# drdeford/FlipComplexityEmpirical

Hardware: AMD Instinct MI355X
Metric: flip steps/sec (whole node), 100×100 grid k=4 batched chains; % HBM peak (higher is better)
Workload: dtype int32

## Files before the change

### flipcomplexityempirical_amd/csrc/fw_grid16.hip

```cpp
#include <hip/hip_runtime.h>

#include <cstdio>
#include <cstdlib>

#include <algorithm>

#include "fw_device.h"

#ifdef FW_STAMPS
__device__ unsigned long long g_stamps[16];
__device__ unsigned long long g_unit_t[2 * 65536];
__device__ unsigned long long g_unit_hw[65536];
#define UNIT_TIME(u, e)                                                         \
  do {                                                                          \
    uint64_t t_;                                                                \
    asm volatile("s_memrealtime %0\n\ts_waitcnt lgkmcnt(0)" : "=s"(t_)::"memory"); \
    if (__lane_id() == 0 && (u) < 65536) {                                      \
      g_unit_t[2 * (u) + (e)] = t_;                                             \
      if ((e) == 0)                                                             \
        g_unit_hw[u] = (unsigned long long)__builtin_amdgcn_s_getreg((31 << 11) | 4) | \
                       ((unsigned long long)__builtin_amdgcn_s_getreg((31 << 11) | 20) << 32); \
    }                                                                           \
  } while (0)
#define STAMP_DECL uint64_t st_acc[16] = {}; uint64_t st_t0 = 0;
#define STAMP(i)                                              \
  do {                                                        \
    __builtin_amdgcn_sched_barrier(0);                        \
    uint64_t st_t1;                                           \
    asm volatile("s_memtime %0\n\ts_waitcnt lgkmcnt(0)" : "=s"(st_t1)::"memory"); \
    __builtin_amdgcn_sched_barrier(0);                        \
    if (i >= 0) st_acc[(i) < 0 ? 0 : (i)] += st_t1 - st_t0;   \
    st_t0 = st_t1;                                            \
  } while (0)
#define STAMP_FLUSH                                           \
  if (__lane_id() == 0)                                       \
    for (int i_ = 0; i_ < 16; ++i_) atomicAdd(&g_stamps[i_], (unsigned long long)st_acc[i_]);
#define STAMP_COUNT(i, v) st_acc[i] += (uint64_t)(v)
#else
#define STAMP_COUNT(i, v)
#define STAMP_DECL
#define STAMP(i)
#define STAMP_FLUSH
#define UNIT_TIME(u, e)
#endif

#include <cstddef>

static_assert(sizeof(fw_chain_stats) == 136, "fw_chain_stats layout");
static_assert(offsetof(fw_chain_stats, yields) == 88 && offsetof(fw_chain_stats, sum_invb) == 112 &&
                  offsetof(fw_chain_stats, cut) == 120 && offsetof(fw_chain_stats, npairs) == 128,
              "fw_chain_stats layout");

#define HIST_ADD(ptr, v) atomicAdd(ptr, v)

void* fw_grid16_pick_lean(int lb, int mode, int G, bool w4);
void* fw_grid16_pick_w2(int mode, int G, bool w4);

namespace {

constexpr int ROW = 16;
constexpr int MAX_NW = 4;
constexpr uint32_t SCR_BLOCK = 15;
constexpr int LDS_GUARD = 16;

struct Hood16 {
  int x;
  uint32_t lx;
  uint32_t bits;
  uint32_t cnt;
  bool has_v;
  int deg;
};

struct GDiv {
  uint32_t m, s;
  __device__ __forceinline__ int operator()(int x) const {
    return (int)(__umul24((uint32_t)x, m) >> s);
  }
};
__device__ __forceinline__ int mulW(int r, int W) { return (int)__umul24((uint32_t)r, (uint32_t)W); }

__device__ __forceinline__ uint32_t rowbits(uint64_t bal, int row) {
  return (uint32_t)(bal >> (row * ROW)) & 0xFFFFu;
}
__device__ __forceinline__ uint32_t row_scan(uint32_t x) {
  x += (uint32_t)__builtin_amdgcn_update_dpp(0, (int)x, 0x111, 0xF, 0xF, true);
  x += (uint32_t)__builtin_amdgcn_update_dpp(0, (int)x, 0x112, 0xF, 0xF, true);
  x += (uint32_t)__builtin_amdgcn_update_dpp(0, (int)x, 0x114, 0xF, 0xF, true);
  x += (uint32_t)__builtin_amdgcn_update_dpp(0, (int)x, 0x118, 0xF, 0xF, true);
  return x;
}
__device__ __forceinline__ uint32_t row_last(uint32_t x) {
  return (uint32_t)__builtin_amdgcn_update_dpp(0, (int)x, 0x15F, 0xF, 0xF, false);
}
__device__ __forceinline__ uint32_t row_sum(uint32_t x) { return row_last(row_scan(x)); }
__device__ __forceinline__ uint32_t row_first(uint32_t x) {
  return (uint32_t)__builtin_amdgcn_update_dpp(0, (int)x, 0x150, 0xF, 0xF, false);
}
__device__ __forceinline__ uint32_t row_shl1(uint32_t x) {
  return (uint32_t)__builtin_amdgcn_update_dpp(0, (int)x, 0x101, 0xF, 0xF, false);
}
__device__ __forceinline__ uint32_t row_pick(uint32_t x, int L, int q) {
  const int src = ((__lane_id() - q) + L) << 2;
  return (uint32_t)__builtin_amdgcn_ds_bpermute(src, (int)x);
}

template <int LB>
__device__ __forceinline__ uint32_t lab_window(const LDS uint8_t* lab, int x) {
  const int bit = (x - 1) * LB;
  const int wi = bit >> 5;
  const LDS uint32_t* w = reinterpret_cast<const LDS uint32_t*>(lab);
  const uint32_t lo0 = w[wi];
  const uint32_t lo = wi >= 0 ? lo0 : 0u;
  const uint32_t hi = w[wi + 1];
  const uint64_t both = ((uint64_t)hi << 32) | lo;
  return (uint32_t)(both >> (uint32_t)(bit - wi * 32)) & ((1u << (6 * LB)) - 1u);
}

template <int LB, int MODE>
__device__ __forceinline__ void weights4(const LDS uint8_t* lab, int x0, int W, int H, int n,
                                         GDiv gd, uint32_t& w4, uint32_t& cd4) {
  constexpr uint32_t M = (1u << LB) - 1u;
  w4 = 0;
  cd4 = 0;
  if (x0 >= n) return;
  const uint32_t own = lab_window<LB>(lab, x0);
  const uint32_t up = x0 + 3 - W >= 0 ? lab_window<LB>(lab, x0 - W) : 0u;
  const uint32_t dn = x0 + W < n ? lab_window<LB>(lab, x0 + W) : 0u;
  const int r0 = gd(x0);
  const int c0 = x0 - mulW(r0, W);
#pragma unroll
  for (int tt = 0; tt < 4; ++tt) {
    int ct = c0 + tt, rt = r0;
    if (ct >= W) {
      ct -= W;
      rt += 1;
    }
    const uint32_t lx = (own >> (LB * (tt + 1))) & M;
    const uint32_t ll = (own >> (LB * tt)) & M;
    const uint32_t lr = (own >> (LB * (tt + 2))) & M;
    const uint32_t lu = (up >> (LB * (tt + 1))) & M, ld = (dn >> (LB * (tt + 1))) & M;
    uint32_t bits = 0, cd = 0;
    if (rt > 0) { bits |= 1u << lu; cd += lu != lx; }
    if (ct > 0) { bits |= 1u << ll; cd += ll != lx; }
    if (ct < W - 1) { bits |= 1u << lr; cd += lr != lx; }
    if (rt < H - 1) { bits |= 1u << ld; cd += ld != lx; }
    uint32_t w = MODE == FW_PROPOSE_CUTEDGE ? cd : (uint32_t)__popc(bits & ~(1u << lx));
    if (x0 + tt >= n) w = cd = 0;
    w4 |= w << (8 * tt);
    cd4 |= cd << (8 * tt);
  }
}

__device__ __forceinline__ uint32_t bsum4(uint32_t v) {
  return (v & 0xFFu) + ((v >> 8) & 0xFFu) + ((v >> 16) & 0xFFu) + (v >> 24);
}

__device__ __forceinline__ uint32_t spread4(uint32_t u) {
  const uint32_t t = ((u << 12) | u) & 0x000F000Fu;
  return ((t << 6) | t) & 0x03030303u;
}
__device__ __forceinline__ uint32_t onehot4(uint32_t s) {
  return __builtin_amdgcn_perm(0u, 0x08040201u, s);
}
__device__ __forceinline__ uint32_t low_bytes(int t) {
  const uint32_t tc = (uint32_t)min(max(t, 0), 4);
  return tc == 4u ? 0xFFFFFFFFu : (1u << (8u * tc)) - 1u;
}
__device__ __forceinline__ uint32_t ne_bytes(uint32_t a, uint32_t b) {
  return ~((a & b) + 0x7F7F7F7Fu) & 0x80808080u;
}
__device__ __forceinline__ uint32_t byte_popc(uint32_t f) {
  const uint32_t t = f - ((f >> 1) & 0x55555555u);
  return (t & 0x33333333u) + ((t >> 2) & 0x33333333u);
}

template <int MODE, bool NEED_CD, bool BATCH = true, bool W4 = false>
__device__ __forceinline__ void weights4_swar(const LDS uint8_t* lab, int x0, int W, int H, int n,
                                              GDiv gd, uint32_t& w4, uint32_t& cd4) {
  w4 = 0;
  cd4 = 0;
  const int xs = x0 < n ? x0 : 0;
  const bool hasU = xs + 3 - W >= 0, hasD = xs + W < n;
  const LDS uint32_t* lw32 = reinterpret_cast<const LDS uint32_t*>(lab);
  const int xw[3] = {xs, hasU ? xs - W : xs, hasD ? xs + W : xs};
  uint32_t wlo[3], whi[3];
  int wbit[3];
#pragma unroll
  for (int t = 0; t < 3; ++t) {
    wbit[t] = (xw[t] - 1) * 2;
    const int wi = wbit[t] >> 5;
    wlo[t] = lw32[wi];
    whi[t] = lw32[wi + 1];
  }
  const int r0 = gd(x0);
  const int c0 = x0 - mulW(r0, W);
  const int tw = W - c0;
  uint32_t mN, mU, mD, mL, mR;
  if constexpr (W4) {
    mN = x0 < n ? 0xFFFFFFFFu : 0u;
    mU = r0 > 0 ? 0xFFFFFFFFu : 0u;
    mD = r0 < H - 1 ? 0xFFFFFFFFu : 0u;
    mL = c0 == 0 ? 0xFFFFFF00u : 0xFFFFFFFFu;
    mR = tw == 4 ? 0x00FFFFFFu : 0xFFFFFFFFu;
  } else {
    const uint32_t t8 = (uint32_t)min(tw, 4) << 3;
    const uint32_t nxt = (uint32_t)(~0ull << t8);
    mN = low_bytes(n - x0);
    mU = r0 > 0 ? 0xFFFFFFFFu : nxt;
    mD = r0 < H - 2 ? 0xFFFFFFFFu : (r0 == H - 2 ? ~nxt : 0u);
    mL = ~((uint32_t)(0xFFull << t8) | (c0 == 0 ? 0xFFu : 0u));
    mR = ~(uint32_t)(0xFFull << (((uint32_t)min(tw, 5) << 3) - 8u));
  }
  if constexpr (BATCH) __builtin_amdgcn_sched_barrier(0);
  uint32_t win[3];
#pragma unroll
  for (int t = 0; t < 3; ++t) {
    const int wi = wbit[t] >> 5;
    const uint64_t both = ((uint64_t)whi[t] << 32) | (wi >= 0 ? wlo[t] : 0u);
    win[t] = (uint32_t)(both >> (uint32_t)(wbit[t] - wi * 32)) & 0xFFFu;
  }
  const uint32_t own = win[0];
  const uint32_t up = hasU ? win[1] : 0u, dn = hasD ? win[2] : 0u;
  const uint32_t o_lo = onehot4(spread4(own)), o_hi = onehot4(spread4(own >> 8));
  const uint32_t L = o_lo;
  const uint32_t O = __builtin_amdgcn_alignbyte(o_hi, o_lo, 1);
  const uint32_t R = __builtin_amdgcn_alignbyte(o_hi, o_lo, 2);
  const uint32_t U = onehot4(spread4(up >> 2)), Dn = onehot4(spread4(dn >> 2));
  if constexpr (MODE != FW_PROPOSE_CUTEDGE) {
    const uint32_t bits = (U & mU) | (L & mL) | (R & mR) | (Dn & mD);
    w4 = byte_popc(bits & ~O & mN);
  }
  if constexpr (NEED_CD || MODE == FW_PROPOSE_CUTEDGE) {
    const uint32_t ne = (ne_bytes(U, O) & mU) >> 7, nl = (ne_bytes(L, O) & mL) >> 7,
                   nr = (ne_bytes(R, O) & mR) >> 7, nd = (ne_bytes(Dn, O) & mD) >> 7;
    cd4 = (ne + nl + nr + nd) & mN;
    if constexpr (MODE == FW_PROPOSE_CUTEDGE) w4 = cd4;
  }
}

template <int LB, int MODE, bool NEED_CD, bool BATCH = true, bool W4 = false>
__device__ __forceinline__ void weights4x(const LDS uint8_t* lab, int x0, int W, int H, int n,
                                          GDiv gd, uint32_t& w4, uint32_t& cd4) {
  if constexpr (LB == 2)
    weights4_swar<MODE, NEED_CD, BATCH, W4>(lab, x0, W, H, n, gd, w4, cd4);
  else
    weights4<LB, MODE>(lab, x0, W, H, n, gd, w4, cd4);
}

__device__ __forceinline__ uint32_t bsum4m(uint32_t v) { return (v * 0x01010101u) >> 24; }


__device__ __forceinline__ int window_verdict8(uint64_t A, int q, int row, bool need, uint32_t& nflood) {
#ifdef FW_STAMPS
#define FLOOD_COUNT ++nflood
#else
#define FLOOD_COUNT
#endif
  constexpr uint64_t BORDER = 0x7Full | (0x7Full << 48) | 0x0001010101010101ull | 0x0040404040404040ull;
  const uint64_t src = A & ((1ull << 19) | (1ull << 26) | (1ull << 28) | (1ull << 35));
  const int sb = q == 0 ? 19 : q == 1 ? 26 : q == 2 ? 28 : 35;
  uint64_t x = (need && q < 4) ? src & (1ull << sb) : 0ull;
  if (x) {
    for (;;) {
      const uint64_t y = (x | (x << 1) | (x >> 1) | (x << 8) | (x >> 8)) & A;
      x = (y | (y << 1) | (y >> 1) | (y << 8) | (y >> 8)) & A;
      FLOOD_COUNT;
      if (x == y) break;
    }
  }
  const uint32_t full = rowbits(ballot(x != 0ull && (x & src) == src), row);
  const uint32_t closed = rowbits(ballot(x != 0ull && (x & BORDER) == 0ull), row);
  return full ? 1 : (closed ? 0 : -1);
}

__device__ __forceinline__ uint32_t from_prev_row_lane(uint32_t x) {
  return (uint32_t)__builtin_amdgcn_update_dpp(0, (int)x, 0x111, 0xF, 0xF, true);
}
__device__ __forceinline__ uint32_t from_next_row_lane(uint32_t x) {
  return (uint32_t)__builtin_amdgcn_update_dpp(0, (int)x, 0x101, 0xF, 0xF, true);
}
__device__ __forceinline__ uint32_t dilate_row(uint32_t x) {
  return x | (x << 1) | (x >> 1) | from_prev_row_lane(x) | from_next_row_lane(x);
}

template <int LB>
__device__ int grid_race_bb_row(const LDS uint8_t* lab, int n, int W, int H, int q, int row,
                                bool need, int vr, int vc, uint32_t a, uint32_t am4, uint32_t lk,
                                uint32_t& nodes, uint32_t& degs) {
  const int r = vr - 8 + q, c0 = vc - 16;
  const bool rin = (r >= 0) & (r < H);
  uint32_t A = eq_bits32<LB>(lab, n, (rin ? r : vr) * W + c0, a);
  const int lo_cut = c0 < 0 ? -c0 : 0;
  const int hi_n = W - c0;
  uint32_t cm = ~0u << lo_cut;
  if (hi_n < 32) cm &= (1u << hi_n) - 1u;
  A &= rin ? cm : 0u;
  if (q == 8) A &= ~(1u << 16);
  uint32_t E = ((q == 0) & (r > 0)) | ((q == 15) & (r < H - 1)) ? ~0u : 0u;
  if (c0 > 0) E |= 1u;
  if (c0 + 31 < W - 1) E |= 1u << 31;
  E &= A;
  uint32_t F[4];
#pragma unroll
  for (int d = 0; d < 4; ++d) {
    const int sl = d == 0 ? 7 : (d == 3 ? 9 : 8), sb = d == 1 ? 15 : (d == 2 ? 17 : 16);
    F[d] = (q == sl && ((am4 >> d) & 1u)) ? (1u << sb) : 0u;
  }
  uint32_t M = 0x8421u;
  auto unite = [&](int i, int j) {
    const uint32_t m = ((M >> (4 * i)) | (M >> (4 * j))) & 15u;
#pragma unroll
    for (int d = 0; d < 4; ++d)
      M = ((m >> d) & 1u) ? (M & ~(15u << (4 * d))) | (m << (4 * d)) : M;
  };
  if (lk & 1u) unite(0, 2);
  if (lk & 2u) unite(2, 3);
  if (lk & 4u) unite(3, 1);
  if (lk & 8u) unite(1, 0);
  auto n_classes = [&]() {
    int nc = 0;
#pragma unroll
    for (int d = 0; d < 4; ++d)
      nc += (int)(((am4 >> d) & 1u) && (__ffs((M >> (4 * d)) & 15u) - 1) == d);
    return nc;
  };
  uint32_t V = F[0] | F[1] | F[2] | F[3];
  int verdict = need ? -2 : -1;
  uint32_t P = 0;
  while (ballot(verdict == -2)) {
    const bool run = verdict == -2;
    const uint32_t lvl = F[0] | F[1] | F[2] | F[3];
    if (run && n_classes() == 1) {
      verdict = 1;
      P = V & ~lvl;
    }
    const bool esc = rowbits(ballot((lvl & E) != 0u), row) != 0u;
    if (verdict == -2 && esc) verdict = -3;
    const bool go = verdict == -2;
    uint32_t D[4], nw = 0;
#pragma unroll
    for (int d = 0; d < 4; ++d) {
      D[d] = ((am4 >> d) & 1u) ? dilate_row(F[d]) & A : 0u;
      nw |= D[d];
    }
    nw &= ~V;
#pragma unroll
    for (int i = 0; i < 4; ++i)
#pragma unroll
      for (int j = i + 1; j < 4; ++j) {
        const bool cand = go && ((am4 >> i) & 1u) && ((am4 >> j) & 1u) && !((M >> (4 * i + j)) & 1u);
        if (rowbits(ballot(cand && (D[i] & (F[j] | (D[j] & nw))) != 0u), row)) unite(i, j);
      }
    uint32_t reach = 0;
#pragma unroll
    for (int d = 0; d < 4; ++d) {
      const uint32_t fd = D[d] & nw;
      F[d] = go ? fd : F[d];
      reach |= rowbits(ballot(fd != 0u), row) ? (1u << d) : 0u;
    }
    if (go) {
      P = V;
      if (n_classes() == 1) {
        verdict = 1;
      } else {
        bool closed = false;
#pragma unroll
        for (int d = 0; d < 4; ++d)
          closed |= ((am4 >> d) & 1u) && (reach & (M >> (4 * d)) & 15u) == 0u;
        if (closed)
          verdict = 0;
        else
          V |= nw;
      }
    }
  }
  if (verdict < 0) return -1;
  const uint32_t pc = (uint32_t)__popc(P);
  uint32_t dg = pc * (uint32_t)((r > 0) + (r < H - 1) + 2);
  if (c0 <= 0) dg -= (P >> (-c0)) & 1u;
  if (hi_n <= 32) dg -= (P >> (hi_n - 1)) & 1u;
  nodes = row_sum(pc);
  degs = row_sum(dg);
  return verdict;
}

__device__ __forceinline__ uint32_t lane_read(uint32_t x, int L) {
  return (uint32_t)__builtin_amdgcn_ds_bpermute(L << 2, (int)x);
}
template <int R>
__device__ __forceinline__ uint32_t grp_sum(uint32_t x, int gb, int q) {
  uint32_t t = 0;
#pragma unroll
  for (int s = 0; s < R; ++s) t += lane_read(x, gb + s * ROW + q);
  return t;
}
template <int R>
__device__ __forceinline__ uint64_t grp_sum64(uint64_t x, int gb, int q) {
  uint64_t t = 0;
#pragma unroll
  for (int s = 0; s < R; ++s)
    t += (uint64_t)lane_read((uint32_t)x, gb + s * ROW + q) |
         ((uint64_t)lane_read((uint32_t)(x >> 32), gb + s * ROW + q) << 32);
  return t;
}

__device__ __forceinline__ void scr_clear(LDS uint8_t* scr, int x) {
  __atomic_fetch_and(PK<4>::word(scr, x), ~(15u << PK<4>::shift(x)), __ATOMIC_RELAXED);
}

template <int LB>
__device__ bool grid_race(const LDS uint8_t* lab, LDS uint8_t* scr, LDS uint32_t* list,
                          GLB uint32_t* spill, int qcap, int W, int H, GDiv gd, int lane,
                          int v, uint32_t a, int m, int src, uint64_t cls, uint64_t& bfs_nodes,
                          uint64_t& bfs_deg) {
  using P = PK<LB>;
  using S = PK<4>;
  auto list_get = [&](int i) -> uint32_t {
    const uint32_t in_lds = list[i < qcap ? i : qcap - 1];
    uint32_t in_hbm = 0;
    if (i >= qcap) in_hbm = spill[i - qcap];
    return i < qcap ? in_lds : in_hbm;
  };
  auto list_put = [&](int i, uint32_t x) {
    if (i < qcap) list[i] = x;
    if (i >= qcap) spill[i - qcap] = x;
  };
  if (lane == 0) S::axor(scr, v, SCR_BLOCK);
  if (lane < m) {
    S::axor(scr, src, 1u + (uint32_t)lane);
    list_put(lane, (uint32_t)src);
  }
  lds_order();
  int nl = m, lb = 0, le = m;
  uint32_t my_deg = 0;
  int verdict = -1;
  for (;;) {
    uint64_t rep = ballot(lane < m && (__ffsll((unsigned long long)cls) - 1) == lane);
    if (__popcll(rep) == 1) {
      verdict = 1;
      break;
    }
    uint64_t pushed_src = 0;
    for (int base = lb; base < le; base += WAVE) {
      const int idx = base + lane;
      const bool act = idx < le;
      const int x = act ? (int)list_get(idx) : 0;
      const uint32_t o = act ? S::get(scr, x) - 1u : 0u;
      const int xr = gd(x);
      const int xc = x - mulW(xr, W);
      if (act) my_deg += (uint32_t)((xr > 0) + (xc > 0) + (xc < W - 1) + (xr < H - 1));
      bfs_nodes += (uint64_t)__popcll(ballot(act));
#pragma unroll
      for (int j = 0; j < 4; ++j) {
        int y = -1;
        if (act) {
          if (j == 0 && xr > 0) y = x - W;
          if (j == 1 && xc > 0) y = x - 1;
          if (j == 2 && xc < W - 1) y = x + 1;
          if (j == 3 && xr < H - 1) y = x + W;
        }
        bool push = false, req = false;
        uint32_t other = 0;
        if (y >= 0 && P::get(lab, y) == a) {
          const uint32_t got = S::claim(scr, y, 0u, 1u + o);
          if (got == 0u) {
            push = true;
          } else if (got - 1u < (uint32_t)m) {
            req = true;
            other = got - 1u;
          }
        }
        const uint64_t pm = ballot(push);
        if (push) list_put(nl + (int)mbcnt(pm), (uint32_t)y);
        nl += __popcll(pm);
        if (pm) {
          for (int si = 0; si < m; ++si)
            pushed_src |= ballot(push && o == (uint32_t)si) ? (1ull << si) : 0ull;
        }
        uint64_t rm = ballot(req && o != other);
        while (rm) {
          const int Lr = __ffsll((unsigned long long)rm) - 1;
          rm &= rm - 1;
          const int o1 = rdl((int32_t)o, Lr), o2 = rdl((int32_t)other, Lr);
          const uint64_t m1 = rdl64(cls, o1), m2 = rdl64(cls, o2);
          if (m1 != m2) {
            const uint64_t nm = m1 | m2;
            if (lane < m && ((nm >> lane) & 1ull)) cls = nm;
          }
        }
      }
      if (nl > qcap) __threadfence_block();
    }
    lds_order();
    lb = le;
    le = nl;
    rep = ballot(lane < m && (__ffsll((unsigned long long)cls) - 1) == lane);
    if (__popcll(rep) == 1) {
      verdict = 1;
      break;
    }
    const bool closed = lane < m && ((rep >> lane) & 1ull) && ((cls & pushed_src) == 0ull);
    if (ballot(closed)) {
      verdict = 0;
      break;
    }
  }
  bfs_deg += wave_sum(my_deg);
  for (int base = 0; base < nl; base += WAVE) {
    const int idx = base + lane;
    if (idx < nl) scr_clear(scr, (int)list_get(idx));
  }
  if (lane == 0) scr_clear(scr, v);
  lds_order();
  return verdict == 1;
}

template <int LB, int MODE, int PER, bool FULL, bool BIG, int R, bool W2 = false, bool W4 = false>
__device__ __forceinline__ void grid16_body(const FwRunParams& p) {
  static_assert(!W4 || LB == 2, "the width flag belongs to the SWAR weights");
  static_assert(PER % 2 == 0, "group sums are read as u16 pairs");
  static_assert(R == 1 || R == 2 || R == 4, "rows per chain");
  static_assert(R == 1 || (!FULL && !BIG), "speculation: lean small-grid kernels only");
  constexpr int CPW = 4 / R;
  extern __shared__ __align__(16) uint8_t smem[];
  __shared__ int32_t s_lock;
  using P = PK<LB>;
  const int lane = __lane_id(), row = lane >> 4, q = lane & 15;
  const int sx = row & (R - 1);
  const int grp = row / R;
  const int gb = grp * R * ROW;
  const bool owner = sx == 0;
  const int wv = (int)(threadIdx.x >> 6);
  const int W = (int)in_vgpr((uint32_t)p.g.gw), H = (int)in_vgpr((uint32_t)p.g.gh);
  const int n = (int)in_vgpr((uint32_t)p.g.n);
  const int D = (int)in_vgpr((uint32_t)p.g.maxdeg), G = (int)in_vgpr((uint32_t)p.G);
  const int k = (int)in_vgpr((uint32_t)p.k);
  LDS uint8_t* const sm = (LDS uint8_t*)smem;
  LDS uint8_t* const lab = sm + LDS_GUARD + (wv * CPW + grp) * p.slot_stride;
  LDS uint32_t* const gsum = reinterpret_cast<LDS uint32_t*>(lab + p.off_gsum);
  LDS uint32_t* const ssum = reinterpret_cast<LDS uint32_t*>(lab + p.off_ssum);
  LDS uint32_t* const lvl1 = BIG ? ssum : gsum;
  LDS uint8_t* const scr = sm + p.off_scr;
  LDS uint32_t* const list = reinterpret_cast<LDS uint32_t*>(sm + p.off_list16);
  GLB uint32_t* const spill = (GLB uint32_t*)(p.spill + (size_t)blockIdx.x * (size_t)n);
  const uint32_t key0 = (uint32_t)p.seed, key1 = (uint32_t)(p.seed >> 32);
  const int GW = (G + 1) >> 1;
  const int SG = (G + 15) >> 4;
  const bool maps_on = FULL && p.m_acc != nullptr;
  const int32_t pop_lo = (int32_t)in_vgpr((uint32_t)(int32_t)max(p.pop_lo, (int64_t)INT32_MIN));
  const int32_t pop_hi = (int32_t)in_vgpr((uint32_t)(int32_t)min(p.pop_hi, (int64_t)INT32_MAX));
  const GDiv gd{in_vgpr(p.g.gm24), in_vgpr(p.g.gs24)};
  const int32_t rule = FULL ? p.accept : FW_ACCEPT_CUT;
  int my_dr, my_dc;
  role_off(q <= 8 ? q : 0, my_dr, my_dc);
  if (LB == 2 && q >= 9 && q <= 12) {
    my_dr = q == 9 ? -2 : (q == 12 ? 2 : 0);
    my_dc = q == 10 ? -2 : (q == 11 ? 2 : 0);
  }
  const uint32_t nb_lanes = q == 0   ? 0x1Eu
                            : q == 1 ? (1u << 9) | (1u << 8) | (1u << 5)
                            : q == 2 ? (1u << 10) | (1u << 8) | (1u << 7)
                            : q == 3 ? (1u << 11) | (1u << 5) | (1u << 6)
                            : q == 4 ? (1u << 12) | (1u << 6) | (1u << 7)
                                     : 0u;
  auto divmod = [&](int x, int& r, int& c) {
    r = gd(x);
    c = x - mulW(r, W);
  };
  STAMP_DECL

  {
    LDS uint32_t* s32 = reinterpret_cast<LDS uint32_t*>(scr);
    for (int i = (int)threadIdx.x; i < p.scr_bytes / 4; i += (int)blockDim.x) s32[i] = 0u;
    if (threadIdx.x == 0) s_lock = 0;
  }
  __syncthreads();
// ... 168 lines not shown
    };
    if (waits_on && first) wcur = wait_draw(p.seed, FW_WAIT_T0, gid, p.wlp[bnodes]);
    observe(first && owner);

    U4 pb = {0u, 0u, 0u, 0u};
    int bpos = ROW;
    uint32_t w2[PER / 2];
    auto read_lvl1 = [&]() {
#pragma unroll
      for (int t = 0; t < PER / 2; ++t) w2[t] = lvl1[q * (PER / 2) + t];
    };
    read_lvl1();

    const bool unit_pop = !FULL || p.g.pop == nullptr;
    const uint32_t psh = (uint32_t)p.prio_shift;
    const uint32_t pstep = ustep >= (2u << psh) ? ustep >> psh : 2u;
    uint32_t pnext = pstep, plev = 0;
    if (psh == 3u && (__builtin_amdgcn_s_getreg((3 << 11) | 4) & 1u) == 0u) plev = 1;
    if (plev == 0) __builtin_amdgcn_s_setprio(3);
    else __builtin_amdgcn_s_setprio(2);
    for (;;) {
      STAMP(-1);
      if (!stuck && (retries >= (uint32_t)p.max_retries || npairs == 0)) stuck = 1;
      const bool act = has && !stuck && n_steps < ustep;
      if (ballot(act) == 0ull) break;
      if (rfl(n_steps) >= pnext) {
        pnext += pstep;
        plev = (plev + 1u) & 3u;
        if (plev == 0) __builtin_amdgcn_s_setprio(3);
        else if (plev == 1) __builtin_amdgcn_s_setprio(2);
        else if (plev == 2) __builtin_amdgcn_s_setprio(1);
        else __builtin_amdgcn_s_setprio(0);
      }

      U4 x;
      if constexpr (R == 1) {
        if (bpos == ROW) {
          if (n_sdeg >= p.fold_at || (s_cut | s_bn) >= p.fold_at) {
            if (q == 0 && has) {
              stp->pop_fail += n_popf;
              stp->contig_fail += n_conf;
              stp->sum_deg += n_sdeg;
              stp->sum_cut += s_cut;
              stp->sum_bnodes += s_bn;
            }
            att0 += n_att;
            n_att = n_popf = n_conf = n_sdeg = 0;
            s_cut = s_bn = 0;
          }
          const uint64_t t = att0 + (uint64_t)(n_att + (uint32_t)q);
          pb = philox((uint32_t)t, (uint32_t)(t >> 32), (uint32_t)gid, (uint32_t)(gid >> 32),
                      in_vgpr(key0), in_vgpr(key1));
          bpos = 0;
        }
        x = U4{row_first(pb.x0), row_first(pb.x1), row_first(pb.x2), row_first(pb.x3)};
        pb = U4{row_shl1(pb.x0), row_shl1(pb.x1), row_shl1(pb.x2), row_shl1(pb.x3)};
        ++bpos;
        n_att += act ? 1u : 0u;
      } else {
        if (bpos_w > (uint32_t)(ROW * R - R)) {
          const uint32_t s_any = lane_read(s_cut | s_bn, gb + q);
          if (4u * n_att >= p.fold_at || s_any >= p.fold_at) {
            const uint32_t f0 = grp_sum<R>(n_popf, gb, q), f1 = grp_sum<R>(n_conf, gb, q);
            const uint32_t f2 = grp_sum<R>(n_sdeg, gb, q);
            if (q == 0 && owner && has) {
              stp->pop_fail += f0;
              stp->contig_fail += f1;
              stp->sum_deg += f2;
              stp->sum_cut += s_cut;
              stp->sum_bnodes += s_bn;
            }
            att0 += n_att;
            n_att = n_popf = n_conf = n_sdeg = 0;
            s_cut = s_bn = 0;
          }
          const uint64_t t = att0 + (uint64_t)(n_att + (uint32_t)(sx * ROW + q));
          pb = philox((uint32_t)t, (uint32_t)(t >> 32), (uint32_t)gid, (uint32_t)(gid >> 32),
                      in_vgpr(key0), in_vgpr(key1));
          bpos_w = 0;
        }
        const int srcl = gb + (int)bpos_w + sx;
        x = U4{lane_read(pb.x0, srcl), lane_read(pb.x1, srcl), lane_read(pb.x2, srcl),
               lane_read(pb.x3, srcl)};
      }
      const uint32_t r = scale64(x.x0, x.x1, (uint32_t)(npairs > 0 ? npairs : 1));

      STAMP(0);
      uint32_t s = 0;
#pragma unroll
      for (int t = 0; t < PER / 2; ++t) s += (w2[t] & 0xFFFFu) + (w2[t] >> 16);
      uint32_t pp[PER / 2];
      {
        uint32_t base = 0;
#pragma unroll
        for (int t = 0; t < PER / 2; ++t) {
          pp[t] = __umul24(base, 0x10001u) + (w2[t] + (w2[t] << 16));
          base = pp[t] >> 16;
        }
      }
      const uint32_t incl = row_scan(s);
      const uint32_t rb1 = rowbits(ballot(incl > r), row);
      const int Lw = __ffs(rb1) - 1;
      const uint32_t rl = r - (incl - s);
      typedef uint16_t u16x2 __attribute__((ext_vector_type(2)));
      const u16x2 rl2 = __builtin_bit_cast(u16x2, __umul24(rl & 0xFFFFu, 0x10001u));
      u16x2 mn = {0xFFFFu, 0xFFFFu}, wraps = {0u, 0u};
#pragma unroll
      for (int t = 0; t < PER / 2; ++t) {
        const u16x2 e = rl2 - __builtin_bit_cast(u16x2, pp[t]);
        mn = __builtin_elementwise_min(mn, e);
        wraps += e >> (uint16_t)15;
      }
      const uint32_t rem = min(rl, (uint32_t)min(mn.x, mn.y));
      const int tfu = PER - (int)wraps.x - (int)wraps.y;
      const int tf = min(tfu, PER - 1);
      const uint32_t pk1 = row_pick(((uint32_t)(q * PER + tf) << 16) | (rem & 0xFFFFu), Lw, q);
      int gi;
      uint32_t r1;
      uint32_t rbg = 1u;
      if constexpr (BIG) {
        const int sgi = min((int)(pk1 >> 16), SG - 1);
        const uint32_t r1s = pk1 & 0xFFFFu;
        const uint32_t g2 = gsum[sgi * 8 + (q >> 1)];
        const uint32_t gv = (q & 1) ? (g2 >> 16) : (g2 & 0xFFFFu);
        const uint32_t incg = row_scan(gv);
        rbg = rowbits(ballot(incg > r1s), row);
        const int Lg = __ffs(rbg) - 1;
        const uint32_t pkg =
            row_pick(((uint32_t)(sgi * 16 + q) << 16) | ((r1s - (incg - gv)) & 0xFFFFu), Lg, q);
        gi = min((int)(pkg >> 16), G - 1);
        r1 = pkg & 0xFFFFu;
      } else {
        gi = min((int)(pk1 >> 16), G - 1);
        r1 = pk1 & 0xFFFFu;
      }

      STAMP(1);
      const int x0 = gi * 64 + q * 4;
      uint32_t w4, cd4;
      weights4x<LB, MODE, false, !W2, W4>(lab, x0, W, H, n, gd, w4, cd4);
      const uint32_t pref1 = w4 + (w4 << 8);
      const uint32_t pref = pref1 + (pref1 << 16);
      const uint32_t ws = pref >> 24;
      const uint32_t incl2 = row_scan(ws);
      const uint32_t rb2 = rowbits(ballot(incl2 > r1), row);
      const int L2 = __ffs(rb2) - 1;
      const uint32_t r2 = min(r1 - (incl2 - ws), 127u);
      const uint32_t gt = ((pref | 0x80808080u) - __builtin_amdgcn_perm(0u, r2 + 1u, 0u)) & 0x80808080u;
      const int t2 = gt ? (__ffs(gt) - 1) >> 3 : 3;
      const uint32_t bef2 = t2 ? (pref >> (8 * t2 - 8)) & 0xFFu : 0u;
      const uint32_t pk2 = row_pick(((uint32_t)(q * 4 + t2) << 16) | ((r2 - bef2) & 0xFFFFu), L2, q);
      const int v = min(gi * 64 + (int)(pk2 >> 16), n - 1);
      const uint32_t j = pk2 & 0xFFFFu;
      if (R == 1 && act && (rb1 == 0 || rb2 == 0 || rbg == 0)) stuck = 2;
      const bool go = act && rb1 != 0 && rb2 != 0 && rbg != 0;

      STAMP(2);
      int vr, vc;
      divmod(v, vr, vc);
      const int dv = (vr > 0) + (vc > 0) + (vc < W - 1) + (vr < H - 1);
      Hood16 h;
      h.x = -1;
      h.lx = NOLAB;
      h.bits = 0;
      h.cnt = 0;
      h.has_v = false;
      h.deg = 0;
      if constexpr (LB == 2) {
        const int xr = vr + my_dr, xc = vc + my_dc;
        const bool inb = (q <= 12) & ((uint32_t)xr < (uint32_t)H) & ((uint32_t)xc < (uint32_t)W);
        const int xx = mulW(xr, W) + xc;
        const uint32_t l0 = P::get(lab, inb ? xx : v);
        h.x = inb ? xx : -1;
        h.lx = inb ? l0 : NOLAB;
        const uint32_t m0 = rowbits(ballot(h.lx == 0u), row) & nb_lanes;
        const uint32_t m1 = rowbits(ballot(h.lx == 1u), row) & nb_lanes;
        const uint32_t m2 = rowbits(ballot(h.lx == 2u), row) & nb_lanes;
        const uint32_t m3 = rowbits(ballot(h.lx == 3u), row) & nb_lanes;
        h.bits = (m0 ? 1u : 0u) | (m1 ? 2u : 0u) | (m2 ? 4u : 0u) | (m3 ? 8u : 0u);
        if constexpr (MODE == FW_PROPOSE_CUTEDGE) {
          const uint32_t same = h.lx == 0u ? m0 : h.lx == 1u ? m1 : h.lx == 2u ? m2 : m3;
          h.cnt = (uint32_t)__popc(m0 | m1 | m2 | m3) - (uint32_t)__popc(same);
          h.deg = q == 0 ? (int)h.cnt + (int)__popc(same) : 0;
        }
        h.has_v = q >= 1 && q <= 4 && inb;
        if (!(inb && q <= 4)) {
          h.bits = 0;
          h.cnt = 0;
        }
      } else {
        const int xr = vr + my_dr, xc = vc + my_dc;
        if (q <= 8 && xr >= 0 && xr < H && xc >= 0 && xc < W) {
          h.x = xr * W + xc;
          h.lx = P::get(lab, h.x);
          if (q <= 4) {
            h.deg = (xr > 0) + (xc > 0) + (xc < W - 1) + (xr < H - 1);
            const int vslot = 4 - q;
#pragma unroll
            for (int jj = 0; jj < 4; ++jj) {
              int y = -1;
              if (jj == 0 && xr > 0) y = h.x - W;
              if (jj == 1 && xc > 0) y = h.x - 1;
              if (jj == 2 && xc < W - 1) y = h.x + 1;
              if (jj == 3 && xr < H - 1) y = h.x + W;
              if (y < 0) continue;
              if (q > 0 && jj == vslot) {
                h.has_v = true;
                continue;
              }
              const uint32_t ly = P::get(lab, y);
              h.bits |= 1u << ly;
              h.cnt += ly != h.lx;
            }
          }
        }
      }
      const uint32_t a = row_first(h.lx);
      const bool isnb = q >= 1 && q <= 4 && h.x >= 0;
      uint32_t d;
      if constexpr (MODE == FW_PROPOSE_CUTEDGE) {
        const uint32_t cm = rowbits(ballot(isnb && h.lx != a), row) >> 1;
        uint32_t mm = cm;
        for (uint32_t t = 0; t < j && t < 4; ++t) mm &= mm - 1;
        const int Lc = __ffs(mm);
        d = row_pick(h.lx, Lc, q);
      } else {
        uint32_t mask;
        if constexpr (LB == 2) {
          mask = row_first(h.bits) & ~(1u << a);
        } else {
          uint32_t fb = (isnb && h.lx != a) ? (1u << h.lx) : 0u;
          fb |= (uint32_t)__builtin_amdgcn_update_dpp(0, (int)fb, 0x111, 0xF, 0xF, true);
          fb |= (uint32_t)__builtin_amdgcn_update_dpp(0, (int)fb, 0x112, 0xF, 0xF, true);
          fb |= (uint32_t)__builtin_amdgcn_update_dpp(0, (int)fb, 0x114, 0xF, 0xF, true);
          mask = (uint32_t)__builtin_amdgcn_update_dpp(0, (int)fb, 0x154, 0xF, 0xF, false);
        }
        uint32_t mm = mask;
        if constexpr (LB == 2) {
          const uint32_t m1 = mm & (mm - 1u), m2 = m1 & (m1 - 1u);
          mm = j == 0u ? mm : (j == 1u ? m1 : m2);
        } else {
          for (uint32_t t = 0; t < j && t < 15; ++t) mm &= mm - 1;
        }
        d = (uint32_t)(__ffs(mm) - 1);
      }
      const uint32_t amb = rowbits(ballot(isnb && h.lx == a), row) >> 1;
      const int m = __popc(amb);
      const int nbd = __popc(rowbits(ballot(isnb && h.lx == d), row) >> 1);
      const int dcut = m - nbd;

      const int32_t pv = unit_pop ? 1 : (int32_t)p.g.pop[v];
      const bool bad = (((uint32_t)q == a) & (pops - pv < pop_lo)) |
                       (((uint32_t)q == d) & (pops + pv > pop_hi));
      const bool pop_ok = rowbits(ballot(bad), row) == 0u;

      STAMP(3);
      uint32_t wo = 0, wn = 0;
      const bool mine = (q <= 4) & (h.x >= 0);
      if constexpr (MODE == FW_PROPOSE_CUTEDGE) {
        const uint32_t wo_v = (uint32_t)(h.deg - m), wn_v = (uint32_t)(h.deg - nbd);
        const uint32_t wo_u = h.cnt + (uint32_t)(h.has_v & (a != h.lx));
        const uint32_t wn_u = h.cnt + (uint32_t)(h.has_v & (d != h.lx));
        wo = q == 0 ? wo_v : wo_u;
        wn = q == 0 ? wn_v : wn_u;
      } else {
        const uint32_t hv = h.has_v ? 0xFFFFFFFFu : 0u;
        const uint32_t ka = q == 0 ? ~(1u << a) : ~(1u << h.lx);
        const uint32_t kd = q == 0 ? ~(1u << d) : ~(1u << h.lx);
        wo = (uint32_t)__popc((h.bits | ((1u << a) & hv)) & ka);
        wn = (uint32_t)__popc((h.bits | ((1u << d) & hv)) & kd);
      }
      wo = mine ? wo : 0u;
      wn = mine ? wn : 0u;
      const uint64_t b_plus = ballot(go && mine && wo == 0 && wn > 0);
      const uint64_t b_minus = ballot(go && mine && wo > 0 && wn == 0);
      const int plus = __popc(rowbits(b_plus, row)), minus = __popc(rowbits(b_minus, row));
      const double invb_new = p.g.invb[bnodes + plus - minus];
      bool wacc = false;
      if constexpr (R > 1) {
        const bool acc_l = (((uint64_t)(x.x2 >> 5) << 26) | (uint64_t)(x.x3 >> 6)) < thr53_l;
        wacc = ((rowbits(ballot(acc_l), row) >> (dcut + D)) & 1u) != 0u;
      }
      uint32_t it_bfs = 0;
      uint64_t it_bfsn = 0, it_bfsd = 0;
      auto count_search = [&](uint64_t bn_, uint64_t bd_) {
        if constexpr (R == 1) {
          n_bfs += 1;
          n_bfsn += bn_;
          n_bfsd += bd_;
        } else {
          it_bfs = 1;
          it_bfsn = bn_;
          it_bfsd = bd_;
        }
      };
      const uint32_t rbits8 = rowbits(ballot(q >= 1 && q <= 8 && h.lx == a), row) >> 1;
      const int pN = rbits8 & 1, pW = (rbits8 >> 1) & 1, pE = (rbits8 >> 2) & 1, pS = (rbits8 >> 3) & 1;
      const int NE = (rbits8 >> 4) & 1, SE = (rbits8 >> 5) & 1, SW = (rbits8 >> 6) & 1,
                NW = (rbits8 >> 7) & 1;
      const int lNE = pN & pE & NE, lES = pE & pS & SE, lSW = pS & pW & SW, lWN = pW & pN & NW;
      bool contig = (m == 1) | ((m >= 2) & (m - (lNE + lES + lSW + lWN) <= 1));
      bool need = go & pop_ok & (m >= 2) & !contig;
      if (ballot(need)) {
        uint64_t A = 0;
        bool inw[4];
        uint32_t raw[4], lw[4];
        int xw[4];
        const int wcol = q & 7;
#pragma unroll
        for (int t = 0; t < 4; ++t) {
          const int wrow = 2 * t + (q >> 3);
          const int rr = vr + wrow - 3, cw = vc + wcol - 3;
          inw[t] = (wcol < 7) & (wrow < 7) & ((uint32_t)rr < (uint32_t)H) & ((uint32_t)cw < (uint32_t)W);
          xw[t] = inw[t] ? mulW(rr, W) + cw : v;
          raw[t] = lab[xw[t] >> 2];
          if constexpr (LB != 2) raw[t] = P::get(lab, xw[t]);
        }
        if constexpr (!W2) __builtin_amdgcn_sched_barrier(0);
#pragma unroll
        for (int t = 0; t < 4; ++t) lw[t] = LB == 2 ? (raw[t] >> ((xw[t] & 3) << 1)) & 3u : raw[t];
#pragma unroll
        for (int t = 0; t < 4; ++t)
          A |= (uint64_t)rowbits(ballot(inw[t] & (lw[t] == a)), row) << (ROW * t);
        A &= ~(1ull << 27);
        uint32_t nflood = 0;
        const int wvd = window_verdict8(A, q, row, need, nflood);
        STAMP_COUNT(12, 1);
        STAMP_COUNT(13, __builtin_amdgcn_readfirstlane(__reduce_max_sync(~0ull, nflood)));
        if (wvd >= 0) {
          contig = wvd == 1;
          need = false;
        }
      }
      STAMP(7);
      if (BIG && !p.no_bb && !p.no_rowbb && ballot(need)) {
        uint32_t bn16 = 0, bd16 = 0;
        const int vb = grid_race_bb_row<LB>(lab, n, W, H, q, row, need, vr, vc, a, amb,
                                            (uint32_t)(lNE | (lES << 1) | (lSW << 2) | (lWN << 3)),
                                            bn16, bd16);
        if (need && vb >= 0) {
          contig = vb == 1;
          need = false;
          count_search(bn16, bd16);
        }
      }
      uint64_t rows_need = ballot(q == 0 && need);
      bool locked = false;
      while (rows_need) {
        const int L0 = __ffsll((unsigned long long)rows_need) - 1;
        rows_need &= rows_need - 1;
        const int rr = L0 >> 4;
        if constexpr (R > 1) {
          if (rr % R) {
            const uint64_t sure = ballot(q == 0 && go && pop_ok && contig && wacc);
            const uint32_t before = (uint32_t)((1u << (rr % R)) - 1u) << (rr - rr % R);
            uint32_t rows_sure = 0;
#pragma unroll
            for (int r4 = 0; r4 < 4; ++r4) rows_sure |= ((sure >> (16 * r4)) & 1u) << r4;
            if (rows_sure & before) continue;
          }
        }
        const uint32_t aa = rdl(a, L0);
        const uint32_t am4 = rdl(amb, L0);
        const uint32_t lk = rdl((uint32_t)(lNE | (lES << 1) | (lSW << 2) | (lWN << 3)), L0);
        uint64_t bn = 0, bd = 0;
        int verdict = -1;
        if (!p.no_bb)
          verdict = grid_race_bb<LB>(sm + LDS_GUARD + (wv * CPW + rr / R) * p.slot_stride, n, W, H,
                                    lane, rdl(vr, L0), rdl(vc, L0), aa, am4, lk, bn, bd);
        if (verdict >= 0) {
          if (row == rr) {
            contig = verdict == 1;
            count_search(bn, bd);
          }
          continue;
        }
        if (!locked) {
          if (lane == 0) {
            int expect = 0;
            while (!__hip_atomic_compare_exchange_strong(&s_lock, &expect, 1, __ATOMIC_ACQUIRE,
                                                         __ATOMIC_RELAXED,
                                                         __HIP_MEMORY_SCOPE_WORKGROUP)) {
              expect = 0;
              __builtin_amdgcn_s_sleep(1);
            }
          }
          lds_order();
          locked = true;
        }
        const int vv = rdl(v, L0);
        const int mr = __popc(am4);
        int srcn = -1;
        uint32_t mm = am4;
        for (int i = 0; i < mr; ++i) {
          const int bit = __ffs(mm) - 1;
          mm &= mm - 1;
          const int val = rdl(h.x, L0 + 1 + bit);
          if (lane == i) srcn = val;
        }
        uint64_t cls = lane < mr ? (1ull << lane) : 0ull;
        auto sx = [&](int b) { return __popc(am4 & ((1u << b) - 1u)); };
        auto merge = [&](int s1, int s2) {
          const uint64_t nm = rdl64(cls, s1) | rdl64(cls, s2);
          if (lane < mr && ((nm >> lane) & 1ull)) cls = nm;
        };
        if (lk & 1) merge(sx(0), sx(2));
        if (lk & 2) merge(sx(2), sx(3));
        if (lk & 4) merge(sx(3), sx(1));
        if (lk & 8) merge(sx(1), sx(0));
        const bool ok = grid_race<LB>(sm + LDS_GUARD + (wv * CPW + rr / R) * p.slot_stride, scr, list, spill,
                                      p.qcap16, W, H, gd, lane, vv, aa, mr, srcn, cls, bn,
                                      bd);
        if (row == rr) {
          contig = ok;
          count_search(bn, bd);
        }
      }
      if (locked && lane == 0)
        __hip_atomic_store(&s_lock, 0, __ATOMIC_RELEASE, __HIP_MEMORY_SCOPE_WORKGROUP);

      STAMP(4);
      const bool valid = go && pop_ok && contig;
      if constexpr (R > 1) {
        const bool accepted = valid && wacc;
        const uint64_t b_go = ballot(q == 0 && go), b_val = ballot(q == 0 && valid);
        const uint64_t b_acc = ballot(q == 0 && accepted);
        uint32_t cons = 0, kold = 0, ns = n_steps, rt = retries;
        int fpos = -1;
        bool stop = !act;
#pragma unroll
        for (int s2 = 0; s2 < R; ++s2) {
          const int L = gb + s2 * ROW;
          const bool g2 = (b_go >> L) & 1ull, v2 = (b_val >> L) & 1ull, a2 = (b_acc >> L) & 1ull;
          if (!stop && !g2) {
            stuck = 2;
            stop = true;
          }
          if (!stop) {
            cons = (uint32_t)s2 + 1u;
            if (v2) {
              ns += 1u;
              rt = 0u;
              if (a2) {
                fpos = s2;
                stop = true;
              } else {
                kold += 1u;
              }
              if (ns >= ustep) stop = true;
            } else {
              rt += 1u;
              if (rt >= (uint32_t)p.max_retries) stop = true;
            }
          }
        }
        if (sx < (int)cons) {
          n_sdeg += (uint32_t)dv;
          if (!pop_ok) n_popf += 1;
          else if (!contig) n_conf += 1;
          n_bfs += it_bfs;
          n_bfsn += it_bfsn;
          n_bfsd += it_bfsd;
        }
        n_steps = ns;
        retries = rt;
        n_att += cons;
        bpos_w += cons;
        const bool commit_me = sx == fpos;
        if (commit_me) {
          n_acc += 1;
          n_adeg += (uint32_t)dv;
          n_bchg += (uint32_t)(plus + minus);
          if (q == 0) P::axor(lab, v, a ^ d);
          if (mine && wn != wo) lds_add(gsum + (h.x >> 7), (wn - wo) << (16 * ((h.x >> 6) & 1)));
        }
        lds_order();
        read_lvl1();
        uint32_t dl = commit_me && mine ? wn - wo : 0u;
        dl += (uint32_t)__builtin_amdgcn_update_dpp(0, (int)dl, 0x111, 0xF, 0xF, true);
        dl += (uint32_t)__builtin_amdgcn_update_dpp(0, (int)dl, 0x112, 0xF, 0xF, true);
        dl += (uint32_t)__builtin_amdgcn_update_dpp(0, (int)dl, 0x114, 0xF, 0xF, true);
        const int dnp = (int)(uint32_t)__builtin_amdgcn_update_dpp(0, (int)dl, 0x154, 0xF, 0xF, false);
        const int fsrc = gb + (fpos < 0 ? 0 : fpos) * ROW + q;
        const uint32_t pk = (uint32_t)(dcut + 8) | ((uint32_t)plus << 4) | ((uint32_t)minus << 8) |
                            (a << 12) | (d << 16) | ((uint32_t)(dnp + 64) << 20);
        const uint32_t pkf = lane_read(pk, fsrc);
        const uint64_t ib = (uint64_t)__double_as_longlong(invb_new);
        const uint32_t ibl = lane_read((uint32_t)ib, fsrc), ibh = lane_read((uint32_t)(ib >> 32), fsrc);
        for (uint32_t i = 0; i < kold; ++i) observe(owner);
        if (fpos >= 0) {
          npairs += (int)((pkf >> 20) & 127u) - 64;
          cut += (int)(pkf & 15u) - 8;
          bnodes += (int)((pkf >> 4) & 15u) - (int)((pkf >> 8) & 15u);
          invb = __longlong_as_double((long long)(((uint64_t)ibh << 32) | ibl));
          if ((uint32_t)q == ((pkf >> 12) & 15u)) pops -= 1;
          if ((uint32_t)q == ((pkf >> 16) & 15u)) pops += 1;
          observe(owner);
        }
        STAMP(5);
        continue;
      }
      if (go) {
        n_sdeg += (uint32_t)dv;
        if (!pop_ok) n_popf += 1;
        else if (!contig) n_conf += 1;
        retries = valid ? 0u : retries + 1u;
      }
      bool accepted;
      if (rule == FW_ACCEPT_BOUNDARY) {
        const int32_t fv = p.flags[v] ? 1 : 0;
        const int32_t cnt = bcnt - ((uint32_t)q == a ? fv : 0) + ((uint32_t)q == d ? fv : 0);
        accepted = valid && __popc(rowbits(ballot(q < k && cnt > 0), row)) >= 2;
      } else {
        bool acc_l;
        if (rule == FW_ACCEPT_BRATIO) {
          const double bound = thr_l * ((double)(bnodes + plus - minus) / (double)bnodes);
          acc_l = u53(x.x2, x.x3) < bound;
        } else {
          acc_l = (((uint64_t)(x.x2 >> 5) << 26) | (uint64_t)(x.x3 >> 6)) < thr53_l;
        }
        accepted = valid & (((rowbits(ballot(acc_l), row) >> (dcut + D)) & 1u) != 0u);
      }
      STAMP(8);
      if (FULL && p.trace != nullptr && valid && q == 0)
        p.trace[(size_t)c * p.steps + n_steps] = accepted ? v * 64 + (int)d : -1;
      n_steps += valid ? 1u : 0u;
      if (maps_on && accepted) {
        const int64_t t = (int64_t)(yields0 + (n_steps - 1u) + (first ? 1u : 0u));
        if (q >= 1 && q <= 4 && h.x >= 0 && (h.lx == a || h.lx == d)) {
          const int e = q == 1   ? grid_eid_down(vr - 1, vc, W, H)
                        : q == 2 ? grid_eid_right(vr, vc - 1, W, H)
                        : q == 3 ? grid_eid_right(vr, vc, W, H)
                                 : grid_eid_down(vr, vc, W, H);
          map_edge(p, c, e, h.lx == a, t);
        }
        if (q == 0) map_run_end(p, c, pend, t);
        pend = Pend{v, (int32_t)d, (uint32_t)t};
      }

      if (accepted) {
        if (q == 0) P::axor(lab, v, a ^ d);
        if (mine && wn != wo) {
          lds_add(gsum + (h.x >> 7), (wn - wo) << (16 * ((h.x >> 6) & 1)));
          if (BIG) lds_add(ssum + (h.x >> 11), (wn - wo) << (16 * ((h.x >> 10) & 1)));
        }
      }
      lds_order();
      read_lvl1();
      uint32_t dl = accepted && mine ? wn - wo : 0u;
      dl += (uint32_t)__builtin_amdgcn_update_dpp(0, (int)dl, 0x111, 0xF, 0xF, true);
      dl += (uint32_t)__builtin_amdgcn_update_dpp(0, (int)dl, 0x112, 0xF, 0xF, true);
      dl += (uint32_t)__builtin_amdgcn_update_dpp(0, (int)dl, 0x114, 0xF, 0xF, true);
      const int dnp = (int)(uint32_t)__builtin_amdgcn_update_dpp(0, (int)dl, 0x154, 0xF, 0xF, false);
      if (FULL && RN && accepted && p.ring_node[v]) {
        const int32_t np2 = ring_pair();
        if (np2 != rpair) {
          if (q == 0 && rrun) atomicAdd(p.hist_ring + rpair, (unsigned long long)rrun);
          rrun = 0;
          rpair = np2;
        }
      }
      STAMP(9);
      asm volatile("" ::"v"(invb_new));
      invb = accepted ? invb_new : invb;
      if (accepted) {
        n_acc += 1;
        if (FULL && p.sched) sched_row(n_acc);
        n_adeg += (uint32_t)dv;
        npairs += dnp;
        cut += dcut;
        bnodes += plus - minus;
        n_bchg += (uint32_t)(plus + minus);
        if ((uint32_t)q == a) pops -= pv;
        if ((uint32_t)q == d) pops += pv;
        if (rule == FW_ACCEPT_BOUNDARY && p.flags[v]) {
          if ((uint32_t)q == a) bcnt -= 1;
          if ((uint32_t)q == d) bcnt += 1;
        }
        if (waits_on) wcur = wait_draw(p.seed, att0 + (uint64_t)(n_att - 1u), gid, p.wlp[bnodes]);
      }
      observe(valid);
      STAMP(5);
    }

    STAMP(6);
    if constexpr (R > 1) {
      n_popf = grp_sum<R>(n_popf, gb, q);
      n_conf = grp_sum<R>(n_conf, gb, q);
      n_sdeg = grp_sum<R>(n_sdeg, gb, q);
      n_acc = grp_sum<R>(n_acc, gb, q);
      n_adeg = grp_sum<R>(n_adeg, gb, q);
      n_bchg = grp_sum<R>(n_bchg, gb, q);
      n_bfs = grp_sum64<R>(n_bfs, gb, q);
      n_bfsn = grp_sum64<R>(n_bfsn, gb, q);
      n_bfsd = grp_sum64<R>(n_bfsd, gb, q);
    }
    if (has && owner) {
      if (hc0) HIST_ADD(p.hist_cut + base_c + q, (unsigned long long)hc0);
      if (hc1) HIST_ADD(p.hist_cut + base_c + ROW + q, (unsigned long long)hc1);
      if (hb0) HIST_ADD(p.hist_b + base_b + q, (unsigned long long)hb0);
      if (hb1) HIST_ADD(p.hist_b + base_b + ROW + q, (unsigned long long)hb1);
      if (FULL && RN && q == 0 && rrun) atomicAdd(p.hist_ring + rpair, (unsigned long long)rrun);
      int qw = q;
      if constexpr (OPQ) asm volatile("" : "+v"(qw));
      u32x4* dst = reinterpret_cast<u32x4*>(p.labels + (size_t)c * p.lab_stride);
      const LDS u32x4* src = reinterpret_cast<const LDS u32x4*>(lab);
      for (int i = qw; i < p.lab_copy16; i += ROW) dst[i] = src[i];
      if (qw < k) p.pops[(size_t)c * k + qw] = (int64_t)pops;
      if (qw < k && rule == FW_ACCEPT_BOUNDARY) p.bcnt[(size_t)c * k + qw] = bcnt;
      if (q == 0 && maps_on) pend_store(p, c, pend);
      if (q == 0 && waits_on) {
        p.wsamp[2 * (size_t)c] = wsum;
        p.wsamp[2 * (size_t)c + 1] = wcur;
      }
      if (q <= 8) {
        int qr = qw;
        if constexpr (!OPQ) asm volatile("" : "+v"(qr));
        uint64_t* rec = reinterpret_cast<uint64_t*>(stp) + 2 * qr;
        const uint64_t o0 = rec[0];
        const uint64_t o1 = qr < 8 ? rec[1] : 0ull;
        const uint64_t yinc = (uint64_t)n_steps + (first ? 1u : 0u);
        uint64_t w0, w1;
        switch (q) {
          case 0: w0 = att0 + n_att; w1 = o1 + n_steps; break;
          case 1: w0 = o0 + n_acc; w1 = o1 + n_popf; break;
          case 2: w0 = o0 + n_conf; w1 = o1 + n_bfs; break;
          case 3: w0 = o0 + n_bfsn; w1 = o1 + n_bfsd; break;
          case 4: w0 = o0 + n_sdeg; w1 = o1 + n_adeg; break;
          case 5: w0 = o0 + n_bchg; w1 = o1 + yinc; break;
          case 6: w0 = o0 + s_cut; w1 = o1 + s_bn; break;
          case 7:
            w0 = (uint64_t)__double_as_longlong(sum_invb);
// ... 384 lines not shown
```

Baseline: 4.264 billion.

## Flood-fill 7x7 contiguity window with per-lane row words and DPP neighbors

Replaces the 64-bit single-lane window flood fill with a row-parallel layout. Each lane loads one window row as two 32-bit LDS words and extracts a 7-bit label-match mask with SWAR. The four seed sources are packed into byte lanes, so one flood propagates all sources at once, using DPP row shifts for vertical neighbors. This cuts the per-flip LDS loads and ballots and parallelizes the flood across lanes. In exchange it adds wave-wide ballot loop termination and more complex verdict logic.

```diff
diff --git a/flipcomplexityempirical_amd/csrc/fw_grid16.hip b/flipcomplexityempirical_amd/csrc/fw_grid16.hip
--- a/flipcomplexityempirical_amd/csrc/fw_grid16.hip
+++ b/flipcomplexityempirical_amd/csrc/fw_grid16.hip
@@ -6,6 +6,7 @@
 #include <algorithm>
 
 #include "fw_device.h"
+#include "fw_window_rows.h"
 
 #ifdef FW_STAMPS
 __device__ unsigned long long g_stamps[16];
@@ -250,29 +251,6 @@
 
 __device__ __forceinline__ uint32_t bsum4m(uint32_t v) { return (v * 0x01010101u) >> 24; }
 
-
-__device__ __forceinline__ int window_verdict8(uint64_t A, int q, int row, bool need, uint32_t& nflood) {
-#ifdef FW_STAMPS
-#define FLOOD_COUNT ++nflood
-#else
-#define FLOOD_COUNT
-#endif
-  constexpr uint64_t BORDER = 0x7Full | (0x7Full << 48) | 0x0001010101010101ull | 0x0040404040404040ull;
-  const uint64_t src = A & ((1ull << 19) | (1ull << 26) | (1ull << 28) | (1ull << 35));
-  const int sb = q == 0 ? 19 : q == 1 ? 26 : q == 2 ? 28 : 35;
-  uint64_t x = (need && q < 4) ? src & (1ull << sb) : 0ull;
-  if (x) {
-    for (;;) {
-      const uint64_t y = (x | (x << 1) | (x >> 1) | (x << 8) | (x >> 8)) & A;
-      x = (y | (y << 1) | (y >> 1) | (y << 8) | (y >> 8)) & A;
-      FLOOD_COUNT;
-      if (x == y) break;
-    }
-  }
-  const uint32_t full = rowbits(ballot(x != 0ull && (x & src) == src), row);
-  const uint32_t closed = rowbits(ballot(x != 0ull && (x & BORDER) == 0ull), row);
-  return full ? 1 : (closed ? 0 : -1);
-}
 
 __device__ __forceinline__ uint32_t from_prev_row_lane(uint32_t x) {
   return (uint32_t)__builtin_amdgcn_update_dpp(0, (int)x, 0x111, 0xF, 0xF, true);
@@ -1047,32 +1025,34 @@
       bool contig = (m == 1) | ((m >= 2) & (m - (lNE + lES + lSW + lWN) <= 1));
       bool need = go & pop_ok & (m >= 2) & !contig;
       if (ballot(need)) {
-        uint64_t A = 0;
-        bool inw[4];
-        uint32_t raw[4], lw[4];
-        int xw[4];
-        const int wcol = q & 7;
-#pragma unroll
-        for (int t = 0; t < 4; ++t) {
-          const int wrow = 2 * t + (q >> 3);
-          const int rr = vr + wrow - 3, cw = vc + wcol - 3;
-          inw[t] = (wcol < 7) & (wrow < 7) & ((uint32_t)rr < (uint32_t)H) & ((uint32_t)cw < (uint32_t)W);
-          xw[t] = inw[t] ? mulW(rr, W) + cw : v;
-          raw[t] = lab[xw[t] >> 2];
-          if constexpr (LB != 2) raw[t] = P::get(lab, xw[t]);
-        }
-        if constexpr (!W2) __builtin_amdgcn_sched_barrier(0);
-#pragma unroll
-        for (int t = 0; t < 4; ++t) lw[t] = LB == 2 ? (raw[t] >> ((xw[t] & 3) << 1)) & 3u : raw[t];
-#pragma unroll
-        for (int t = 0; t < 4; ++t)
-          A |= (uint64_t)rowbits(ballot(inw[t] & (lw[t] == a)), row) << (ROW * t);
-        A &= ~(1ull << 27);
-        uint32_t nflood = 0;
-        const int wvd = window_verdict8(A, q, row, need, nflood);
+        const int wr = vr - 3 + q;
+        const bool rin = (q < 7) & ((uint32_t)wr < (uint32_t)H);
+        const int wbit = (mulW(rin ? wr : vr, W) + vc - 3) * LB;
+        const int wi = wbit >> 5;
+        const LDS uint32_t* lw32 = reinterpret_cast<const LDS uint32_t*>(lab);
+        const uint32_t wlo = lw32[wi], whi = lw32[wi + 1];
+        uint32_t cm = win_col_mask(vc, W);
+        cm = q == 3 ? cm & ~8u : cm;
+        cm = (rin & need) ? cm : 0u;
+        const uint32_t A4 = (win_row_mask<LB>(wlo, whi, (uint32_t)wbit & 31u, a) & cm) * 0x01010101u;
+        uint32_t fx = win_seed(q, amb) & A4;
+        [[maybe_unused]] uint32_t nflood = 0;
+        for (;;) {
+          const uint32_t fy = win_dilate(fx, from_prev_row_lane(fx), from_next_row_lane(fx), A4);
+          fx = win_dilate(fy, from_prev_row_lane(fy), from_next_row_lane(fy), A4);
+          ++nflood;
+          if (!ballot(fx != fy)) break;
+        }
+        const uint32_t ex4 = win_exist4(amb);
+        uint32_t vt = win_touch(fx, q) | (win_miss(fx, ex4) ? 1u : 0u);
+        vt |= (uint32_t)__builtin_amdgcn_update_dpp(0, (int)vt, 0x111, 0xF, 0xF, true);
+        vt |= (uint32_t)__builtin_amdgcn_update_dpp(0, (int)vt, 0x112, 0xF, 0xF, true);
+        vt |= (uint32_t)__builtin_amdgcn_update_dpp(0, (int)vt, 0x114, 0xF, 0xF, true);
+        vt = (uint32_t)__builtin_amdgcn_update_dpp(0, (int)vt, 0x156, 0xF, 0xF, false);
+        const int wvd = win_verdict((vt & 1u) != 0u, vt, ex4);
         STAMP_COUNT(12, 1);
-        STAMP_COUNT(13, __builtin_amdgcn_readfirstlane(__reduce_max_sync(~0ull, nflood)));
-        if (wvd >= 0) {
+        STAMP_COUNT(13, nflood);
+        if (need & (wvd >= 0)) {
           contig = wvd == 1;
           need = false;
         }
diff --git a/flipcomplexityempirical_amd/csrc/fw_window_rows.h b/flipcomplexityempirical_amd/csrc/fw_window_rows.h
--- /dev/null
+++ b/flipcomplexityempirical_amd/csrc/fw_window_rows.h
@@ -0,0 +1,69 @@
+#pragma once
+#include <stdint.h>
+
+#if defined(__HIPCC__) || defined(__CUDACC__)
+#define FW_WR_FN __host__ __device__ inline
+#else
+#define FW_WR_FN inline
+#endif
+
+template <int LB>
+FW_WR_FN uint32_t win_row_mask(uint32_t lo, uint32_t hi, uint32_t sh, uint32_t a) {
+  static_assert(LB == 2 || LB == 3 || LB == 4, "window rows: 2-, 3- or 4-bit labels");
+  const uint32_t x = (uint32_t)((((uint64_t)hi << 32) | lo) >> sh);
+  uint32_t e;
+  if (LB == 2) {
+    const uint32_t y = x ^ (a * 0x1555u);
+    e = ~(y | (y >> 1)) & 0x1555u;
+    e = (e | (e >> 1)) & 0x3333u;
+    e = (e | (e >> 2)) & 0x0F0Fu;
+    e = e | (e >> 4);
+  } else if (LB == 3) {
+    const uint32_t y = x ^ (a * 0x49249u);
+    e = ~(y | (y >> 1) | (y >> 2)) & 0x49249u;
+    e = (e | (e >> 2)) & 0xC30C3u;
+    e = (e | (e >> 4)) & 0xF00Fu;
+    e = e | (e >> 8);
+  } else {
+    const uint32_t y = x ^ (a * 0x1111111u);
+    e = ~(y | (y >> 1) | (y >> 2) | (y >> 3)) & 0x1111111u;
+    e = (e | (e >> 3)) & 0x03030303u;
+    e = (e | (e >> 6)) & 0x000F000Fu;
+    e = e | (e >> 12);
+  }
+  return e & 0x7Fu;
+}
+
+FW_WR_FN uint32_t win_col_mask(int vc, int W) {
+  const int lo = 3 - vc, hi = vc + 4 - W;
+  return (0x7Fu << (lo > 0 ? lo : 0)) & (0x7Fu >> (hi > 0 ? hi : 0)) & 0x7Fu;
+}
+
+FW_WR_FN uint32_t win_seed(int q, uint32_t amb) {
+  const uint32_t up = (amb & 1u) << 3, lf = ((amb >> 1) & 1u) << (8 + 2);
+  const uint32_t rt = ((amb >> 2) & 1u) << (16 + 4), dn = ((amb >> 3) & 1u) << (24 + 3);
+  return q == 2 ? up : q == 3 ? (lf | rt) : q == 4 ? dn : 0u;
+}
+
+FW_WR_FN uint32_t win_exist4(uint32_t amb) {
+  return (((amb & 15u) * 0x00204081u) & 0x01010101u) * 0xFFu;
+}
+
+FW_WR_FN uint32_t win_dilate(uint32_t x, uint32_t above, uint32_t below, uint32_t A4) {
+  return (x | (x << 1) | (x >> 1) | above | below) & A4;
+}
+
+FW_WR_FN uint32_t win_miss(uint32_t x, uint32_t E4) {
+  const uint32_t u = (x | (x >> 8) | (x >> 16) | (x >> 24)) & 0x7Fu;
+  return (x ^ (u * 0x01010101u)) & E4;
+}
+
+FW_WR_FN uint32_t win_touch(uint32_t x, int q) {
+  const uint32_t b = (q == 0 || q == 6) ? 0x7F7F7F7Fu : 0x41414141u;
+  return ((x & b) + 0x7F7F7F7Fu) & 0x80808080u;
+}
+
+FW_WR_FN int win_verdict(bool miss, uint32_t touch, uint32_t E4) {
+  if (!miss) return 1;
+  return (E4 & 0x80808080u & ~touch) ? 0 : -1;
+}
```

Result: faster. 4.425 billion, median of 6 (+3.8%).
